# thorstone25/qups

Measured on AMD Instinct MI355X. Metric: beamformed Mpixels/sec (1024^2 px, 256x256 Tx/Rx), higher is better.
Workload: dtype f32; 1 GPU; C3: 256-el FSA (256 Tx x 256 Rx), 1024x1024 ScanCartesian lambda/4, T=2816, complex64, lanczos3; pixels=1048576, pairs_per_frame=68719476736, kernel=tiled, reciprocal_mode=True, reciprocity_fold=True, mirror_mode=True, kernel_name=das_tile_kernel<interp=3,f32,sym,fold,mirror,mb=32,W=128> [jit 56fb2bda29f94d0f], jit=True, fallback_tiles=0, aperture_split=1, parallelism=1 GPU, device=AMD Radeon Graphics (gfx950:sramecc+:xnack-), cu=256

## Files before the change

qups_amd/csrc/das_tile_impl.h:

```cpp
#pragma once
#include "tile_params.h"
#ifndef QDAS_DBG_SYNC
#define QDAS_DBG_SYNC 0
#endif
#ifndef QDAS_ONEACC_PLAIN
#define QDAS_ONEACC_PLAIN 0
#endif
#ifndef QDAS_F16_PIPE
#define QDAS_F16_PIPE 0
#endif
#include "tile_util.h"
#include "tile_taps.h"
#include "tile_hooks.h"
#include "das_tile_cfg.h"

namespace qdas {

typedef __attribute__((address_space(3))) void lds_void;

template <int INTERP_, typename ST_, bool FMOD_, bool WTAB_, bool SYM_, bool FB2_, bool FB4_, int WAVES_, int MB_, int W_, int NBUF_, bool BIG_, bool LUT_, bool BF_ = false, bool MIRQ_ = false, bool FOLD_ = false>
struct TileCfg {
    static constexpr int INTERP = INTERP_, WAVES = WAVES_, MB = MB_, W = W_, NBUF = NBUF_;
    using ST = ST_;
    static constexpr bool FMOD = FMOD_, WTAB = WTAB_, SYM = SYM_, FB2 = FB2_, FB4 = FB4_, BIG = BIG_, LUT = LUT_;
// ... 64 lines not shown
    uint32_t split, S, tile_id;
    uint32_t Sm, sm;
    double fs, symC; int symCi;
    bool tile_interior;
    int need_b;
    static constexpr uint32_t NOT_MINE = 0xffffffffu;
    uint32_t pofs;
    __device__ __forceinline__ bool in_shard() const { return pofs != NOT_MINE; }
    static __device__ __forceinline__ uint32_t lane_now() {
        uint32_t l;
        asm volatile("v_mbcnt_lo_u32_b32 %0, -1, 0\n\tv_mbcnt_hi_u32_b32 %0, -1, %0" : "=v"(l));
        return l;
    }
    uint64_t ipx;
    uint64_t ipx2;
    GT px, py, pz;
    double cf;
    uint32_t n_lo, n_hi, nstage;
    uint32_t nact; bool use_act;
    v2f acc, acc1, acc2, acc3;
    v2f ra[C::MB / 2];
    v2f bw[C::BPIX ? C::MB / 2 : 1]; bool bp;
    double rad[C::F64 ? C::MB : 1];
    double dacc[4];
    v2f tot[C::NFR];
    double dtot[2], w64[2];
    bool wpix, syn;
    int wb[C::WPW], wb2[C::WPW];
    int qo[C::MIRQ ? (C::FOLD ? 2 * C::WPW : 4) : 1];
    uint32_t soff, soff2;
    __amdgpu_buffer_rsrc_t rsD, rsM;
    uint64_t offD, offM, xbytes;
    int fa, fb;

    __device__ __forceinline__ Tile(const TileParams &p) : P(p) {}

    __device__ __forceinline__ void setup(unsigned char *smem);
    __device__ __forceinline__ uint32_t locate(uint32_t &i1, uint32_t &col, bool first, bool image = false);
    template <bool PROBE> __device__ __forceinline__ bool prologue();
    __device__ __forceinline__ void plan_stages();
    template <bool CHECK> __device__ __forceinline__ void run();
    __device__ __forceinline__ void epilogue();

    __device__ __forceinline__ uint32_t blk(uint32_t r) const {
        if constexpr (C::SYM) return (r * S + ((r & 1u) ? S - 1u - split : split)) * C::MB;
        else if constexpr (C::ACT) return (r * Sm + sm) * C::MB;
        else return r * C::MB;
    }
    __device__ __forceinline__ uint32_t nlim(uint32_t m0) const { return C::SYM ? (m0 + C::MB < N ? m0 + C::MB : N) : n_hi; }

    static __device__ __forceinline__ double dsqrt(double d2) {
        const float s0 = __builtin_amdgcn_sqrtf((float)d2);
        const double sd = (double)s0;
        const double r = __builtin_fma(-sd, sd, d2);
        return __builtin_fma(r, (double)(0.5f * __builtin_amdgcn_rcpf(fmaxf(s0, 1.0e-30f))), sd);
    }
    __device__ __forceinline__ double a_of(uint32_t m, const GT *gPv, const GT *gNv) const;
    __device__ __forceinline__ double b_at(GT ex, GT ey, GT ez) const;
    __device__ __forceinline__ double s_at(uint32_t n, GT ex, GT ey, GT ez) const;
    __device__ __forceinline__ bool on_side(uint32_t n, GT ex, GT ey, GT ez) const;
    __device__ __forceinline__ const GT *geo_Pi() const { return (const GT *)P.Pi; }
    __device__ __forceinline__ const GT *geo_Pr() const { return (const GT *)P.Pr; }
    __device__ __forceinline__ const GT *geo_Pv() const { return (const GT *)P.Pv; }
    __device__ __forceinline__ const GT *geo_Nv() const { return (const GT *)P.Nv; }
    struct wraw { uint32_t a, b; };
    __device__ __forceinline__ wraw wload_raw(uint32_t n, bool image = false) const;
    __device__ __forceinline__ v2f wconv(wraw r) const;
    __device__ __forceinline__ v2f wload(uint32_t n) const { return wconv(wload_raw(n)); }

    __device__ __forceinline__ __amdgpu_buffer_rsrc_t make_rs(uint64_t o, uint64_t extra) const;
    __device__ __forceinline__ int wjr(int r) const;
    __device__ __forceinline__ void dma_block(uint32_t m0);
    __device__ __forceinline__ void stage_dma(int bn, int buf);
// ... 265 lines not shown
                }
                act[N] = make_uint2(cnt, 0u);
            }
            __syncthreads();
            nact = (uint32_t)__builtin_amdgcn_readfirstlane((int)act[N].x);
            __syncthreads();
        }
    }
    nstage = 0;
    if (use_act) { for (uint32_t r = 0; blk(r) < M; ++r) nstage += nact; }
    else { for (uint32_t r = 0; blk(r) < M; ++r) nstage += nlim(blk(r)) - n_lo; }
}

template <class C> template <bool CHECK> __device__ __forceinline__ void Tile<C>::run() {
    constexpr int NBUF = C::NBUF, NDMA = C::NDMA;
    auto nsel = [&](uint32_t k) -> uint32_t { if constexpr (C::ACT) { if (use_act) return (uint32_t)__builtin_amdgcn_readfirstlane((int)act[k < N ? k : N - 1].x); } return n_lo + k; };
    auto klim = [&](uint32_t mm) -> uint32_t { if constexpr (C::ACT) { if (use_act) return nact; } return nlim(mm) - n_lo; };
    v2f wcur = {1.f, 0.f}, wcur2 = {1.f, 0.f};
    wraw wnext_r = {0x3f800000u, 0u}, wnext_r2 = {0x3f800000u, 0u};
    const uint32_t n_first = nstage ? nsel(0) : n_lo;
    bool wmir = false;
    if constexpr (C::WMIR) wmir = wpix && QSPEC(MIR, P.mir) && QSPEC(HAS_APIX, P.apix != nullptr) && QSPEC(GEN_KIND, P.gen_kind) == 0;
    auto wload64 = [&](uint32_t nn, double &wr, double &wi) {
        const uint64_t k = ipx + (P.apix_pixel_only ? 0ull : P.I1 * P.I2 * P.I3 * (uint64_t)nn);
        if (P.apix_real) { wr = ((const double *)P.apix)[k]; wi = 0.0; }
        else { const double2 v = ((const double2 *)P.apix)[k]; wr = v.x; wi = v.y; }
    };
    double w64n[2] = {1.0, 0.0};
    if constexpr (C::W64) { if (wpix) wload64(n_first, w64[0], w64[1]); }
    else if (wpix) { wcur = wload(n_first); wcur2 = wcur; if constexpr (C::WMIR) { if (wmir) wcur2 = wconv(wload_raw(n_first, true)); } }
    float tbc = 0.f, tbn = 0.f;
    const uint64_t Ilut = P.i_begin + P.i_count;
    if constexpr (C::LUT) tbc = P.lut_rx[ipx + Ilut * n_first];
    uint32_t pr = 0, pk = 0, pm0 = blk(0);
    dma_block(pm0);
    auto rec_base = [&](uint32_t k) -> float { if constexpr (C::F64) return __int_as_float(nrec64[k].b); else return nrec[k].x; };
    float vbn; uint32_t vpn;
    auto front_entry = [&](uint32_t kk) {
        if constexpr (C::ACT) {
            if (use_act) { const uint2 e = act[kk < N ? kk : N - 1]; vpn = e.x; vbn = __uint_as_float(e.y); return; }
        }
        const uint32_t q = n_lo + kk;
        vpn = q; vbn = rec_base(q < N ? q : N - 1);
    };
    front_entry(0);
    int dbn = 0; uint32_t dpn = 0;
    auto dma_prep = [&]() {
        dbn = __builtin_amdgcn_readfirstlane(__float_as_int(vbn));
        dpn = (uint32_t)__builtin_amdgcn_readfirstlane((int)vpn);
        front_entry(pk + 1 == klim(pm0) ? 0u : pk + 1);
    };
    auto dma_go = [&](int buf) {
        if constexpr (C::ACT) {
            if (use_act) {
                soff = ((dpn >> P.stage_shift) - (n_lo >> P.stage_shift)) * (uint32_t)strN * (uint32_t)C::SB;
                if constexpr (C::WMIR) { if (QSPEC(MIR, P.mir)) soff2 = (n_hi - 1u - dpn) * (uint32_t)strN * (uint32_t)C::SB; }
            }
        }
        stage_dma(dbn, buf);
        if (++pk == klim(pm0)) { pk = 0; pm0 = blk(++pr); dma_block(pm0); }
    };
    auto dma_next = [&](int buf) { dma_prep(); dma_go(buf); };
    constexpr uint32_t WBUF = 2u * C::MB * 8u + 16u;
    float2 wnx = {0.f, 0.f};
    auto wst_load = [&](uint32_t nn, uint32_t mm0) {
        if constexpr (C::WST) {
// ... 19 lines not shown
#pragma unroll
    for (int b = 0; b < NBUF - 1; ++b)
        if ((uint32_t)b < nstage) dma_next(b);
    if (nstage >= (uint32_t)(NBUF - 1)) asm volatile("s_waitcnt vmcnt(%0)\n\ts_barrier" ::"n"((NBUF - 2) * NDMA) : "memory");
    else asm volatile("s_waitcnt vmcnt(0)\n\ts_barrier" ::: "memory");
    int buf = 0;
    uint32_t cr = 0, k = 0, n = n_first, m0 = blk(0);
    for (uint32_t st = 0; st < nstage; ++st) {
        timer.mark(0);
        if constexpr ((QDAS_DBG_SYNC & 1) != 0) __syncthreads();
        const bool more = st + (NBUF - 1) < nstage;
        const uint32_t n_next = (NBUF == 2 && C::ACT) ? (uint32_t)__builtin_amdgcn_readfirstlane((int)vpn) : nsel(k + 1 == klim(m0) ? 0u : k + 1);
        const bool skip = wpix && (__ballot(wcur.x != 0.f || wcur.y != 0.f || (C::WMIR && (wcur2.x != 0.f || wcur2.y != 0.f))) == 0ull);
        int rec_b; GT rec_x, rec_y, rec_z;
        if constexpr (C::F64) { const rec64 r = nrec64[n]; rec_b = r.b; rec_x = r.x; rec_y = r.y; rec_z = r.z; }
        else { const float4 r = nrec[n]; rec_b = __float_as_int(r.x); rec_x = r.y; rec_y = r.z; rec_z = r.w; }
        float phB = 0.f;
        if constexpr (C::FMOD && !C::F64) {
            phB = Bext[n];
            if constexpr (C::MIRQ) phB = __uint_as_float((uint32_t)__builtin_amdgcn_readfirstlane((int)__float_as_uint(phB)));
        }
        uint64_t wmask = ~0ull, xmask = ~0ull;
        if constexpr (C::WST) {
            const uint4 mk = *(const uint4 *)(wst + (uint32_t)buf * WBUF + 2 * C::MB * 8);
            wmask = (uint64_t)(uint32_t)__builtin_amdgcn_readfirstlane((int)mk.x) | ((uint64_t)(uint32_t)__builtin_amdgcn_readfirstlane((int)mk.y) << 32);
            if constexpr (C::SYM) xmask = (uint64_t)(uint32_t)__builtin_amdgcn_readfirstlane((int)mk.z) | ((uint64_t)(uint32_t)__builtin_amdgcn_readfirstlane((int)mk.w) << 32);
        }
        const bool dma_late = C::SYM && !hooks::no_late_dma && wave < C::WAVES / 2;
        const bool dma_now = !hooks::no_stage_dma && more && !dma_late;
        if (dma_now) dma_prep();
        if constexpr (C::W64) { if (wpix && st + 1 < nstage) wload64(n_next, w64n[0], w64n[1]); }
        else if (wpix && st + 1 < nstage) { wnext_r = wload_raw(n_next); if constexpr (C::WMIR) { if (wmir) wnext_r2 = wload_raw(n_next, true); } }
        if constexpr (C::LUT) { if (st + 1 < nstage) tbn = P.lut_rx[ipx + Ilut * n_next]; }
        if (st + 1 < nstage) wst_load(n_next, k + 1 == klim(m0) ? blk(cr + 1) : m0);
        if (dma_now) dma_go((buf + NBUF - 1) % NBUF);
        if constexpr ((QDAS_DBG_SYNC & 32) != 0) asm volatile("s_waitcnt vmcnt(0) lgkmcnt(0)" ::: "memory");
        if constexpr ((QDAS_DBG_SYNC & 2) != 0) { asm volatile("s_waitcnt vmcnt(0) lgkmcnt(0)" ::: "memory"); __syncthreads(); }
        timer.mark(1);
        if constexpr (C::F64) {
            if (k == 0) {
#pragma unroll
                for (int p = 0; p < C::MB; ++p) {
                    const uint32_t ma = m0 + p < M ? m0 + p : M - 1;
                    rad[p] = block_residual64(px, py, pz, cf, fs, kindB, (lds_cdouble *)PvL, (lds_cdouble *)NvL, ma, Abase[ma], tapinfo<C::INTERP>::OFF);
                    __builtin_amdgcn_sched_barrier(0);
                }
            }
        } else if (k == 0) {
#pragma unroll
            for (int p = 0; p < C::MB / 2; ++p) {
                const uint32_t ma = m0 + 2 * p < M ? m0 + 2 * p : M - 1, mb = m0 + 2 * p + 1 < M ? m0 + 2 * p + 1 : M - 1;
                if constexpr (C::SYM) {
                    const float4 ea = nrec[ma], eb = nrec[mb];
                    const double fc = symC - (double)symCi - 0.5;
                    ra[p] = (v2f){(float)(b_at(ea.y, ea.z, ea.w) - (double)__float_as_int(ea.x) + fc),
                                  (float)(b_at(eb.y, eb.z, eb.w) - (double)__float_as_int(eb.x) + fc)};
                } else if constexpr (C::LUT)
                    ra[p] = (v2f){(float)(a_of(ma, nullptr, nullptr) - ((double)Abase[ma] + 0.5)), (float)(a_of(mb, nullptr, nullptr) - ((double)Abase[mb] + 0.5))};
                else
                    ra[p] = (v2f){block_residual(px, py, pz, cf, fs, kindB, (lds_cfloat *)PvL, (lds_cfloat *)NvL, ma, Abase[ma], tapinfo<C::INTERP>::OFF),
                                  block_residual(px, py, pz, cf, fs, kindB, (lds_cfloat *)PvL, (lds_cfloat *)NvL, mb, Abase[mb], tapinfo<C::INTERP>::OFF)};
                __builtin_amdgcn_sched_barrier(0);
            }
            if constexpr (C::BPIX) {
                if (!bp) {
#pragma unroll
                    for (int p = 0; p < C::MB / 2; ++p) bw[p] = (v2f){1.f, 1.f};
                } else {
                    const uint64_t Itot = P.I1 * P.I2 * P.I3;
                    uint32_t ip32 = (uint32_t)ipx;
                    asm volatile("" : "+v"(ip32));
#pragma unroll
                    for (int p = 0; p < C::MB / 2; ++p) {
                        const uint32_t ma = m0 + 2 * p < M ? m0 + 2 * p : M - 1, mb = m0 + 2 * p + 1 < M ? m0 + 2 * p + 1 : M - 1;
                        const float *rowa = P.bpix + Itot * ma, *rowb = P.bpix + Itot * mb;
                        asm volatile("" : "+s"(rowa), "+s"(rowb));
                        bw[p] = (v2f){rowa[ip32], rowb[ip32]};
                        __builtin_amdgcn_sched_barrier(0);
                    }
                }
            }
        }
        timer.mark(2);
        if constexpr ((QDAS_DBG_SYNC & 4) != 0) __syncthreads();
        if constexpr (C::F64) {
            const int bn = rec_b;
            const double rbd = s_at(n, rec_x, rec_y, rec_z) - (double)bn;
            const uint32_t cbase = win_off + (uint32_t)buf * (C::NW * C::WB);
            bool skip64 = false;
            if constexpr (C::W64) skip64 = wpix && __ballot(w64[0] != 0.0 || w64[1] != 0.0) == 0ull;
            if (skip64) {}
            else if (m0 + C::MB <= M) pairs_f64<CHECK, false>(n, m0, bn, rbd, cbase);
            else                      pairs_f64<CHECK, true>(n, m0, bn, rbd, cbase);
        } else if (!skip) {
            const int bn = rec_b;
            const float rb = C::LUT ? tbc - (float)bn : hooks::fake_rx_delay ? (float)(lane * 2 + 3) + 0.37f * (float)(n & 7)
                                                                            : (float)(s_at(n, rec_x, rec_y, rec_z) - (double)bn);
            const uint32_t cbase = win_off + (uint32_t)buf * (C::NW * C::WB) - (MAGIC_BITS * (uint32_t)C::SB);
            if (C::SYM ? (n < m0 && (!C::FOLD || m0 + C::MB <= M)) : (m0 + C::MB <= M)) {
                if constexpr (C::TWO && (C::F32 || C::SYM || QDAS_F16_PIPE) && C::K == 4 && !(CHECK || C::FMOD || C::WTAB) && !hooks::no_pipeline && !((QDAS_ONEACC_PLAIN || C::INTERP == 3) && C::ONEACC))
                    pairs_pipelined(rb, cbase);
                else
                {
                    constexpr uint64_t FULL = C::MB >= 64 ? ~0ull : ((1ull << (C::MB & 63)) - 1ull);
                    bool done = false;
                    if constexpr (C::WST) {
                        if (wmask == FULL && (!C::SYM || xmask == FULL)) {
                            pairs_plain<CHECK, false, false>(n, m0, bn, rb, cbase, phB, wst_off + (uint32_t)buf * WBUF, wmask, xmask);
                            done = true;
                        }
                    }
                    if (!done) pairs_plain<CHECK, false>(n, m0, bn, rb, cbase, phB, wst_off + (uint32_t)buf * WBUF, wmask, xmask);
                }
            } else {
                pairs_plain<CHECK, true>(n, m0, bn, rb, cbase, phB, wst_off + (uint32_t)buf * WBUF, wmask, xmask);
            }
        }
        if constexpr ((QDAS_DBG_SYNC & 8) != 0) __syncthreads();
        if constexpr (!hooks::no_fair_prio) __builtin_amdgcn_s_setprio(3);
        if (!hooks::no_stage_dma && more && dma_late) dma_next((buf + NBUF - 1) % NBUF);
        if (st + 1 < nstage) wst_store((buf + 1) % NBUF);
        timer.mark(3);
        if (!hooks::no_stage_barrier) {
            if (more) asm volatile("s_waitcnt vmcnt(%0) lgkmcnt(0)\n\ts_barrier" ::"n"((NBUF - 2) * NDMA) : "memory");
            else asm volatile("s_waitcnt vmcnt(0) lgkmcnt(0)\n\ts_barrier" ::: "memory");
        }
        timer.mark(4);
        timer.stage_done();
        buf = (buf + 1 == NBUF) ? 0 : buf + 1;
        if (syn) {
// ... 5 lines not shown
                if (in_shard()) {
                    float2 *plane = (float2 *)P.y + (size_t)f * P.y_fstride + (size_t)n * P.y_ld;
                    asm volatile("" : "+s"(plane));
                    uint32_t po = pofs;
                    asm volatile("" : "+v"(po));
                    float *q = (float *)(plane + po);
                    unsafeAtomicAdd(q, Sf[f].x); unsafeAtomicAdd(q + 1, Sf[f].y);
                }
            }
            if (wpix) { if constexpr (!C::F32) asm volatile("" : "+v"(wnext_r.a)); wcur = wconv(wnext_r); }
            acc = acc1 = acc2 = acc3 = (v2f){0.f, 0.f};
        } else if (C::W64 && wpix) {
            if constexpr (C::W64) {
                const double sr = dacc[0] + dacc[2], si = dacc[1] + dacc[3];
                dtot[0] += w64[0] * sr - w64[1] * si; dtot[1] += w64[0] * si + w64[1] * sr;
                dacc[0] = dacc[1] = dacc[2] = dacc[3] = 0.0;
                w64[0] = w64n[0]; w64[1] = w64n[1];
            }
        } else if (wpix) {
            v2f Sf[4];
            frame_sums(Sf);
#pragma unroll
            for (int f = 0; f < C::NFR; ++f) {
                const v2f wf = (C::WMIR && f == 1) ? wcur2 : wcur;
                tot[f] += (v2f){wf.x * Sf[f].x - wf.y * Sf[f].y, wf.x * Sf[f].y + wf.y * Sf[f].x};
            }
            acc = acc1 = acc2 = acc3 = (v2f){0.f, 0.f};
            if constexpr (!C::F32) asm volatile("" : "+v"(wnext_r.a));
            wcur = wconv(wnext_r);
            wcur2 = wcur;
            if constexpr (C::WMIR) { if (wmir) { asm volatile("" : "+v"(wnext_r2.a)); wcur2 = wconv(wnext_r2); } }
        }
        if constexpr (C::LUT) tbc = tbn;
        if (++k == klim(m0)) { k = 0; m0 = blk(++cr); }
        n = n_next;
    }
}

template <class C> __device__ __forceinline__ void Tile<C>::epilogue() {
    if (syn || C::BF) return;
    if constexpr (C::F64) {
        if (pofs != NOT_MINE) {
            uint32_t po = pofs;
            asm volatile("" : "+v"(po));
            ST *base = S > 1 ? (ST *)P.part + (size_t)split * P.i_count : (ST *)P.y;
            asm volatile("" : "+s"(base));
            if (C::W64 && wpix) st(base, (size_t)po, cplx<double>{dtot[0], dtot[1]});
            else st(base, (size_t)po, cplx<double>{dacc[0] + dacc[2], dacc[1] + dacc[3]});
        }
    } else {
        v2f res[4];
        frame_sums(res);
        uint32_t po = pofs;
        if constexpr (C::SYM) { uint32_t i1, col; po = locate(i1, col, false); }
        if constexpr (C::FOLDQ && C::FB2) {
            uint32_t i1, col;
            const uint32_t po2 = locate(i1, col, false, true);
            const uint32_t pos[2] = {po, po2};
#pragma unroll
            for (int f = 0; f < 2; ++f) {
#pragma unroll
                for (int h = 0; h < 2; ++h) {
                    uint32_t q = pos[h];
                    if (q == NOT_MINE) continue;
                    asm volatile("" : "+v"(q));
                    const v2f r = res[2 * f + h];
// ... 12 lines not shown
                for (int f = 0; f < 2; ++f) {
                    uint32_t q = pos[f];
                    if (q == NOT_MINE) continue;
                    asm volatile("" : "+v"(q));
                    v2f r = res[f];
                    if constexpr (!C::MIRQ) { if (wpix) r = tot[f]; }
                    if (S > 1) { float2 *base = P.part + (size_t)split * (P.i_count << (QSPEC(MIR, P.mir) == 2 ? 1 : 0)); asm volatile("" : "+s"(base)); base[q] = make_float2(r.x, r.y); }
                    else { ST *base = (ST *)P.y; asm volatile("" : "+s"(base)); st(base, (size_t)q, cplx<float>{r.x, r.y}); }
                }
                return;
            }
        }
        if (po != NOT_MINE) {
            asm volatile("" : "+v"(po));
#pragma unroll
            for (int f = 0; f < C::NFR; ++f) {
                const v2f r = wpix ? tot[f] : res[f];
                if (S > 1) { float2 *base = P.part + ((size_t)split * C::NFR + f) * P.i_count; asm volatile("" : "+s"(base)); base[po] = make_float2(r.x, r.y); }
                else { ST *base = (ST *)P.y + (size_t)f * P.y_fstride; asm volatile("" : "+s"(base)); st(base, (size_t)po, cplx<float>{r.x, r.y}); }
            }
        }
    }
}

template <class C, bool PROBE> __device__ __forceinline__ void das_tile_body(const TileParams &P, unsigned char *smem) {
    Tile<C> t(P);
    t.timer.begin();
    t.setup(smem);
    if (!t.template prologue<PROBE>()) return;
    if constexpr (!PROBE) {
        t.timer.prologue_done();
        t.plan_stages();
        if (P.pro_mask == 2) return;
        if (t.tile_interior) t.template run<false>(); else t.template run<true>();
        t.timer.finish(t.lane, t.wave, C::WAVES);
        t.epilogue();
    }
}

template <int INTERP, typename ST, bool FMOD, bool WTAB, bool SYM, bool FB2, bool FB4, int WAVES, int MB, int W, int NBUF, int PSZ, int BPC, bool PROBE, bool BIG = false, bool LUT = false, bool BFM = false, bool MIRQ = false, bool FOLD = false>
__global__ void __launch_bounds__(WAVES * 64, WAVES * BPC / 4)
das_tile_kernel(const TileParams P) {
    static_assert(PSZ == 16, "16-byte DMA pieces");
    extern __shared__ __attribute__((aligned(16))) unsigned char smem[];
    das_tile_body<TileCfg<INTERP, ST, FMOD, WTAB, SYM, FB2, FB4, WAVES, MB, W, NBUF, BIG, LUT, BFM, MIRQ, FOLD>, PROBE>(P, smem);
}

#ifndef __HIPCC_RTC__
}
#include "jit.h"
namespace qdas {
void tile_census(int ci, int interp, int sample_bytes, bool fm, bool wt, bool probe);
bool tile_prepare_only();
template <int INTERP, typename ST, int CI>
static hipError_t launch_tile_i(const TileParams &P, unsigned ntiles, size_t lds, hipStream_t s) {
    constexpr Cfg G = CFGS[CI];
    constexpr bool FOLD = (CI >= 17 && CI <= 21);
    constexpr bool MIRQ = (CI == 15 || CI == 16 || CI == 17 || CI == 18 || CI == 20);
    constexpr bool SYM = (CI == 1 || CI == 7 || CI == 8 || MIRQ || FOLD), FB2 = (CI == 3 || CI == 4 || CI == 20 || CI == 21), FB4 = (CI == 5 || CI == 6), BIG = (CI == 9), LUT = (CI == 10 || CI == 11), BFM = (CI == 12);
    const bool fm = P.fmod != 0.0, wt = P.wtab != nullptr;
    const dim3 g(ntiles * (P.probe ? 1u : P.ksplit)), b(G.waves * 64);
    tile_census(CI, INTERP, (int)sizeof(ST), fm, wt, P.probe != 0);
#define QDAS_LAUNCH(FM, WT) QDAS_LAUNCH_P(FM, WT, false)
#define QDAS_LAUNCH_P(FM, WT, PR)                                                                        \
    do {                                                                                                 \
        if constexpr (tile_prebuilt(CI, INTERP, FM, WT, PR)) {                                           \
// ... 56 lines not shown
```

qups_amd/csrc/qdas_api.hip:

```cpp
#include <hip/hip_runtime.h>
#include <hip/hip_fp16.h>

#include <algorithm>
#include <cmath>
#include <cstdarg>
#include <cstdio>
#include <cstdlib>
#include <cstring>
#include <string>
#include <mutex>
#include <vector>

#include "../../include/qdas.h"
#include "qdas_kernels.h"
#include "jit.h"

using namespace qdas;

static thread_local std::string g_err;

static int fail(int code, const char *fmt, ...) {
    char buf[512];
    va_list ap;
    va_start(ap, fmt);
// ... 28 lines not shown
    int prev = -1;
    bool restore = false;
    hipError_t err = hipSuccess;
    explicit DeviceGuard(int dev) {
        if (dev < 0) return;
        err = hipGetDevice(&prev);
        if (err == hipSuccess && prev != dev) { err = hipSetDevice(dev); restore = err == hipSuccess; }
    }
    ~DeviceGuard() { if (restore) (void)hipSetDevice(prev); }
    DeviceGuard(const DeviceGuard &) = delete;
    DeviceGuard &operator=(const DeviceGuard &) = delete;
};

static size_t real_size(int dtype) { return dtype == QDAS_F64 ? 8 : 4; }
static size_t data_size(int dtype) { return dtype == QDAS_F64 ? 16 : (dtype == QDAS_F32 ? 8 : 4); }
static size_t apod_real_size(int dtype) { return dtype == QDAS_F64 ? 8 : (dtype == QDAS_F32 ? 4 : 2); }

struct qdas_plan {
    qdas_desc d{};
    uint64_t I = 0, i_count = 0, y_ld = 0, oN = 1, oM = 1;
    double cinv0 = 0.0;
    int device = 0;
    int kernel = QDAS_KERNEL_GENERIC;
    std::vector<void *> owned;
    GenericParams gp{};
    TileParams tp{};
    TileConfig tc{};
    unsigned ntiles = 0, tile_cols = 0;
    bool no_fallback = false;
    double misfit_frac = 0.0;
    bool wtab_real = false;
    void *fold_buf = nullptr;
    const void *fold_wtab = nullptr;
    double mirror_bound = -1.0, recip_bound = -1.0;
    bool prefolded = false;
    qdas_plan *f16_child = nullptr;
    void *y32 = nullptr;
    bool fb2_ok = false;
    bool fb4_off = false;
    bool fold2_ok = false;
    void *fold_buf2 = nullptr;
    qdas_plan *frames_twin = nullptr;
    bool twin_tried = false;
    uint32_t *fallback = nullptr;
    size_t jit_lds = 0;
    int jit_mb = 0, jit_w = 0;
    int hint_mb = 0, hint_w = 0;
    hipFunction_t jit_fn = nullptr;
    std::string jit_tag;
    bool prep2 = false, prep4 = false;
    bool timing = false;
    hipEvent_t e0 = nullptr, e1 = nullptr;
    float last_ms = 0.f;
    void *dx = nullptr, *dy = nullptr;
    size_t x_bytes = 0, y_bytes = 0;
    void *dx2 = nullptr, *dy2 = nullptr;
    hipStream_t copy_stream = nullptr;
    hipEvent_t ex[2] = {nullptr, nullptr}, ek[2] = {nullptr, nullptr};

    ~qdas_plan() {
        if (frames_twin) qdas_plan_destroy(frames_twin);
        if (f16_child) qdas_plan_destroy(f16_child);
        for (void *p : owned) (void)hipFree(p);
        if (e0) (void)hipEventDestroy(e0);
        if (e1) (void)hipEventDestroy(e1);
        for (int k = 0; k < 2; ++k) { if (ex[k]) (void)hipEventDestroy(ex[k]); if (ek[k]) (void)hipEventDestroy(ek[k]); }
// ... 929 lines not shown
    t.pro_mask = 0;
    const bool with_mask = t.act_bytes != 0 && !getenv("QDAS_NO_PRO_MASK");
    const size_t stride = 2 * ((size_t)t.M + t.N) + 8 + (with_mask ? (t.N + 31) / 32 : 0), bytes = (size_t)pl->ntiles * stride * sizeof(float);
    if (bytes > (1ull << 30)) return QDAS_OK;
    void *buf = nullptr;
    if (hipMalloc(&buf, bytes) != hipSuccess) { (void)hipGetLastError(); return QDAS_OK; }
    pl->owned.push_back(buf);
    TileParams p = t;
    p.probe = 1; p.x = nullptr; p.y = nullptr; p.wtab = nullptr; p.apix = nullptr; p.pro_out = (float *)buf; p.pro_mask = with_mask ? 1 : 0;
    HIPCHK(hipMemsetAsync(buf, 0, bytes, 0));
    const hipError_t e = launch_tile(p, pl->d.sz.dtype, pl->ntiles, nullptr);
    if (e != hipSuccess) { (void)hipGetLastError(); return QDAS_OK; }
    HIPCHK(hipStreamSynchronize(nullptr));
    HIPCHK(hipMemset(pl->fallback, 0, sizeof(uint32_t)));
    t.pro_tab = (const float *)buf;
    t.pro_mask = with_mask ? 3 : 0;
    return QDAS_OK;
}

static void plan_cache_activity(qdas_plan *pl) {
    TileParams &t = pl->tp;
    if (pl->kernel != QDAS_KERNEL_TILED || t.pro_mask != 3) return;
    TileParams p = t;
    p.nfr = 1; p.x = nullptr; p.y = nullptr; p.ksplit = 1; p.ksplit_m = 1; p.part = nullptr; p.pro_mask = 2; p.pro_out = const_cast<float *>(t.pro_tab);
    const std::string keep = g_err;
    hipError_t e = launch_tile(p, pl->d.sz.dtype, pl->ntiles, nullptr, pl->jit_fn, pl->jit_lds);
    if (e == hipSuccess) e = hipStreamSynchronize(nullptr);
    if (e == hipSuccess && !pl->no_fallback) e = hipMemset(pl->fallback, 0, sizeof(uint32_t));
    g_err = keep;
    if (e == hipSuccess) t.pro_mask = 1;
    else { (void)hipGetLastError(); t.pro_mask = 0; t.pro_tab = nullptr; }
}

static int plan_build_tiled(qdas_plan *pl, const qdas_desc *desc, PlanBuild &b) {
    int rc;
    if ((rc = plan_setup_tile_params(pl, desc, b))) return rc;
    if ((rc = plan_pixel_weights(pl, desc, b))) return rc;
    if ((rc = plan_weight_table(pl, desc, b))) return rc;
    if ((rc = plan_probe_chain(pl, desc, b))) return rc;
    if ((rc = plan_side_split(pl, desc, b))) return rc;
    if ((rc = plan_wide_windows(pl, desc, b))) return rc;
    if ((rc = plan_stage_shape(pl, desc, b))) return rc;
    if ((rc = plan_split_aperture(pl, b))) return rc;
    if ((rc = plan_cache_prologue(pl))) return rc;
    b.outcome.ksplit = pl->tp.ksplit;
    const modes::LaunchShape model = modes::derive_launch_shape(*desc, b.rq, b.sy, b.outcome), built = launch_shape(pl->tp, pl->d.sz.dtype, false);
    if (const char *f = modes::shape_mismatch(model, built))
        return fail(QDAS_EINVAL, "internal: the built plan differs from the mode model of plan_modes.h in '%s' -- please report the descriptor", f);
    return QDAS_OK;
}

static int plan_create_impl(qdas_plan *pl, qdas_plan **out, const qdas_desc *desc, bool *replaced) {
    *replaced = false;
    int rc = plan_init(pl, desc);
    if (rc) return rc;
    const qdas_sizes &z = pl->d.sz;
    DeviceGuard guard(desc->device);
    if (guard.err != hipSuccess) return fail(QDAS_EHIP, "hipSetDevice(%d): %s", desc->device, hipGetErrorString(guard.err));
    { hipError_t e = hipGetDevice(&pl->device); if (e != hipSuccess) return fail(QDAS_EHIP, "hipGetDevice: %s", hipGetErrorString(e)); }
    if (pl->I == 0 || z.N == 0 || z.M == 0) return QDAS_OK;
    if ((desc->plan_flags & QDAS_PLAN_PREFOLDED) && z.S > 0)
        return fail(QDAS_EUNSUPPORTED, "QDAS_PLAN_PREFOLDED: apodization arrays belong to the fold (qdas_fold_desc.wtab), not to the plan that is handed folded frames");
    PlanBuild b;
    b.desc = desc;
    b.sw = read_switches();
    if ((rc = plan_import_inputs(pl, desc, b))) return rc;
    if ((rc = plan_resolve_modes(pl, desc, b))) return rc;
    if (pl->kernel == QDAS_KERNEL_TILED && (rc = plan_build_tiled(pl, desc, b))) return rc;
    const bool mslab = (desc->plan_flags & QDAS_PLAN_MIRROR_SLAB) != 0;
    if (mslab && !(pl->kernel == QDAS_KERNEL_TILED && pl->tp.mir == 2))
        return fail(QDAS_EUNSUPPORTED, "QDAS_PLAN_MIRROR_SLAB: the lateral-mirror mode is not available for this problem (geometry not mirror-symmetric "
                                       "about x = 0, weights / modes it does not take, or tiles that do not fit the staging windows): use plain slabs");
    int remake = 0;
    if ((rc = plan_jit(pl, desc, &remake))) return rc;
    if (remake) {
        qdas_desc d2 = *desc;
        d2.plan_flags |= remake;
        const std::string keep = g_err;
        *replaced = true;
        const int rc2 = qdas_plan_create(out, &d2);
        if (rc2 == QDAS_OK) g_err = keep;
        return rc2;
    }
    if (pl->prefolded && pl->kernel == QDAS_KERNEL_TILED && !pl->no_fallback)
        return fail(QDAS_EUNSUPPORTED, "QDAS_PLAN_PREFOLDED: tiles of this image do not fit the staging windows (they would be redone from the unfolded frame)");
    plan_f16_child(pl, desc);
    bool no_compiler = false;
    plan_resolve_kernel(pl, &no_compiler);
    if (no_compiler) {
        const std::string why = g_err;
        if (desc->kernel == QDAS_KERNEL_TILED || mslab || pl->prefolded) return fail(QDAS_EUNSUPPORTED, "%s", why.c_str());
        qdas_desc d2 = *desc;
        d2.kernel = QDAS_KERNEL_GENERIC;
        *replaced = true;
        const int rc2 = qdas_plan_create(out, &d2);
        if (rc2 == QDAS_OK) g_err = why + " -- using the generic kernel";
        return rc2;
    }
    plan_cache_activity(pl);
    return plan_finish(pl, desc, b);
}

extern "C" int qdas_plan_create(qdas_plan **out, const qdas_desc *desc) {
    if (!out || !desc) return fail(QDAS_EINVAL, "null argument");
    *out = nullptr;
    int rc = validate(desc);
    if (rc) return rc;
    qdas_plan *pl = new qdas_plan();
    bool replaced = false;
    rc = plan_create_impl(pl, out, desc, &replaced);
    if (rc || replaced) { delete pl; return rc; }
    *out = pl;
    return QDAS_OK;
}

extern "C" void qdas_plan_destroy(qdas_plan *pl) {
    if (!pl) return;
    DeviceGuard guard(pl->device);
    delete pl;
}

extern "C" int qdas_plan_kernel(const qdas_plan *pl) { return pl ? pl->kernel : 0; }

extern "C" int qdas_plan_fallback_tiles(const qdas_plan *pl, uint64_t *n) {
    if (!pl || !n) return fail(QDAS_EINVAL, "null argument");
    if (pl->f16_child) return qdas_plan_fallback_tiles(pl->f16_child, n);
    *n = 0;
    if (pl->kernel != QDAS_KERNEL_TILED || !pl->fallback) return QDAS_OK;
    uint32_t c = 0;
    HIPCHK(hipMemcpy(&c, pl->fallback, sizeof c, hipMemcpyDeviceToHost));
    *n = c;
    return QDAS_OK;
}

extern "C" int qdas_plan_tile_shape(const qdas_plan *pl, int *tile_z, int *tile_cols, int *wave_z, int *ksplit) {
    if (!pl || !tile_z || !tile_cols) return fail(QDAS_EINVAL, "null argument");
    if (pl->f16_child) return qdas_plan_tile_shape(pl->f16_child, tile_z, tile_cols, wave_z, ksplit);
    const bool tiled = pl->kernel == QDAS_KERNEL_TILED;
    *tile_z = tiled ? (1 << pl->tp.tz_log2) : 0;
    *tile_cols = tiled ? (int)pl->tile_cols : 0;
    if (wave_z) *wave_z = tiled ? (1 << pl->tp.wz_log2) : 0;
    if (ksplit) *ksplit = tiled ? (int)pl->tp.ksplit : 0;
    return QDAS_OK;
}

extern "C" int qdas_plan_mirror(const qdas_plan *pl) { if (pl && pl->f16_child) return qdas_plan_mirror(pl->f16_child); return pl && pl->kernel == QDAS_KERNEL_TILED && pl->tp.mir ? 1 : 0; }

extern "C" int qdas_plan_reciprocal(const qdas_plan *pl) { return pl && pl->kernel == QDAS_KERNEL_TILED && pl->tp.sym ? 1 : 0; }

extern "C" int qdas_plan_symmetry_bound(const qdas_plan *pl, double *mirror_samples, double *reciprocal_samples) {
    if (!pl) return fail(QDAS_EINVAL, "null plan");
    if (pl->f16_child) return qdas_plan_symmetry_bound(pl->f16_child, mirror_samples, reciprocal_samples);
    const bool tiled = pl->kernel == QDAS_KERNEL_TILED;
    if (mirror_samples) *mirror_samples = (tiled && pl->tp.mir) ? pl->mirror_bound : -1.0;
    if (reciprocal_samples) *reciprocal_samples = (tiled && pl->tp.sym) ? pl->recip_bound : -1.0;
    return QDAS_OK;
}

extern "C" int qdas_plan_folded(const qdas_plan *pl) { if (pl && pl->f16_child) return 1; return pl && pl->kernel == QDAS_KERNEL_TILED && pl->tp.fold ? 1 : 0; }

extern "C" int qdas_fold(const qdas_fold_desc *d, const void *x, void *xs, void *stream) {
    if (!d || !x || !xs) return fail(QDAS_EINVAL, "null argument");
    if (d->dtype != QDAS_F32 && d->dtype != QDAS_F16) return fail(QDAS_EINVAL, "qdas_fold: complex64 or complex32 (fp16) frames");
    if (d->N > 65535) return fail(QDAS_EUNSUPPORTED, "qdas_fold: at most 65535 elements");
    DeviceGuard guard(d->device);
    HIPCHK(guard.err);
    HIPCHK(launch_fold(x, xs, d->wtab, d->T, d->N, d->strN ? d->strN : d->T, d->strM ? d->strM : d->T * d->N, (hipStream_t)stream, d->dtype == QDAS_F16));
    return QDAS_OK;
}

extern "C" int qdas_plan_kernel_name(const qdas_plan *pl, char *buf, size_t len) {
    if (!pl || !buf || !len) return fail(QDAS_EINVAL, "null argument");
    if (pl->f16_child) {
        char tmp[256];
        int rc = qdas_plan_kernel_name(pl->f16_child, tmp, sizeof tmp);
        if (rc) return rc;
        std::string nm(tmp);
        const size_t at = nm.find(",f32");
        if (at != std::string::npos) nm.replace(at, 4, ",f16>f32");
        if (pl->fold_wtab && nm.find(",wtab") == std::string::npos) { const size_t f = nm.find(",fold"); if (f != std::string::npos) nm.insert(f + 5, ",wtab"); }
        snprintf(buf, len, "%s", nm.c_str());
        return QDAS_OK;
    }
    const qdas_sizes &z = pl->d.sz;
    const char *dts = z.dtype == QDAS_F64 ? "f64" : (z.dtype == QDAS_F32 ? "f32" : "f16");
    if (pl->kernel == QDAS_KERNEL_TILED) {
        const TileParams &t = pl->tp;
        snprintf(buf, len, "das_tile_kernel<interp=%d,%s%s%s%s%s%s%s,mb=%d,W=%d> [%s]", z.flag & 7, dts, t.sym ? ",sym" : "", t.fold ? ",fold" : "", t.fmod != 0.0 ? ",fmod" : "",
                 (t.wtab || (t.fold && pl->fold_wtab)) ? ",wtab" : "", t.big ? ",big" : "", t.mir ? ",mirror" : ((t.St && !t.syn) ? ",roles swapped" : ""), pl->jit_fn ? pl->jit_mb : pl->tc.mb, (pl->jit_fn && pl->jit_w) ? pl->jit_w : pl->tc.window, pl->jit_tag.empty() ? "prebuilt" : pl->jit_tag.c_str());
    } else snprintf(buf, len, "das_generic_kernel<interp=%d,%s>", z.flag & 7, dts);
    return QDAS_OK;
}

extern "C" int qdas_plan_set_timing(qdas_plan *pl, int enable) {
    if (!pl) return fail(QDAS_EINVAL, "null plan");
    pl->timing = enable != 0;
    if (pl->timing && !pl->e0) { HIPCHK(hipEventCreate(&pl->e0)); HIPCHK(hipEventCreate(&pl->e1)); }
    return QDAS_OK;
}

extern "C" int qdas_plan_last_kernel_ms(const qdas_plan *pl, float *ms) {
    if (!pl || !ms) return fail(QDAS_EINVAL, "null argument");
    *ms = pl->last_ms;
    return QDAS_OK;
}

static int hip_rc(hipError_t e) { HIPCHK(e); return QDAS_OK; }

static int run_frame(qdas_plan *pl, const void *x, void *y, hipStream_t s, int nf = 1, uint64_t x_fstride = 0, uint64_t y_fstride = 0) {
    const qdas_sizes &z = pl->d.sz;
    if (pl->f16_child && nf == 1) {
        const TileParams &c = pl->f16_child->tp;
        HIPCHK(launch_fold(x, pl->fold_buf, pl->fold_wtab, z.T, z.N, c.strN, c.strM, s, 1));
        int rc = run_frame(pl->f16_child, pl->fold_buf, pl->y32, s);
        if (rc) return rc;
        HIPCHK(launch_y32_to_y16(pl->y32, y, pl->f16_child->y_ld, s));
        return QDAS_OK;
    }
    if (pl->kernel == QDAS_KERNEL_TILED) {
        TileParams t = pl->tp;
        t.x = x; t.y = y;
        t.nfr = nf; t.x_fstride = x_fstride; t.y_fstride = y_fstride;
        if (t.fold && pl->prefolded) {
            if (!pl->no_fallback) return fail(QDAS_EUNSUPPORTED, "QDAS_PLAN_PREFOLDED: tiles of this image do not fit the staging windows and would need the unfolded frame");
        } else if (t.fold) {
            HIPCHK(launch_fold(x, pl->fold_buf, pl->fold_wtab, z.T, z.N, t.strN, t.strM, s));
            t.x = pl->fold_buf;
            if (nf == 2) {
                if (!pl->fold_buf2) return fail(QDAS_EINVAL, "internal: no second fold buffer");
                HIPCHK(launch_fold((const char *)x + x_fstride, pl->fold_buf2, pl->fold_wtab, z.T, z.N, t.strN, t.strM, s));
                t.x_fstride = (uint64_t)((intptr_t)pl->fold_buf2 - (intptr_t)pl->fold_buf);
            }
        }
        if (t.syn) {
            const size_t ds = data_size(z.dtype);
            for (int f = 0; f < nf; ++f)
                HIPCHK(hipMemset2DAsync((char *)y + (size_t)f * y_fstride * ds, (size_t)pl->y_ld * ds, 0, (size_t)pl->i_count * ds, pl->oN * pl->oM, s));
        }
        const hipFunction_t jf = nf == 1 ? pl->jit_fn : nullptr;
        if (pl->no_fallback) return hip_rc(launch_tile(t, z.dtype, pl->ntiles, s, jf, pl->jit_lds));
        HIPCHK(hipMemsetAsync(pl->fallback, 0, sizeof(uint32_t), s));
        HIPCHK(launch_tile(t, z.dtype, pl->ntiles, s, jf, pl->jit_lds));
        GenericParams g = pl->gp;
        g.x = x; g.y = y; g.y_ld = pl->y_ld;
        g.tile_list = pl->fallback;
        g.tile_cols = pl->tile_cols;
        g.tile_zl = (uint32_t)pl->tp.tz_log2;
        g.blocks_per_tile = (64 * pl->tc.waves + 255) / 256;
        g.tiles_z = pl->tp.tiles_z;
        HIPCHK(launch_generic(g, z.dtype, pl->ntiles * g.blocks_per_tile, s));
        for (int f = 1; f < nf; ++f) {
            g.x = (const char *)x + (size_t)f * x_fstride; g.y = (char *)y + (size_t)f * y_fstride * data_size(z.dtype);
            HIPCHK(launch_generic(g, z.dtype, pl->ntiles * g.blocks_per_tile, s));
        }
    } else {
// ... 807 lines not shown
```

qups_amd/csrc/tile_params.h:

```cpp
#pragma once
#include "tile_rtc.h"

namespace qdas {

struct TileParams {
    const float *Pi, *Pr, *Pv, *Nv, *St;
    int32_t kindB, kindS;
    int32_t stage_shift;
    const void *x;
    void *y;
    const void *wtab;
    const void *apix;
    int32_t apix_real;
    int32_t apix_pixel_only;
    int32_t gen_kind;
    double gen_p0, gen_p1;
    const float *rxn;
    uint32_t act_bytes;
    uint64_t T, N, M, I1, I2, I3;
    uint64_t i_begin, i_count;
    uint64_t strN, strM;
    double cinv_fs;
    const float *cinv_pix;
    double fs, fmod;
    int32_t flag, VS, DV;
    int32_t narrow;
    int32_t big;
    int32_t sym;
    int32_t tz_log2;
    int32_t wz_log2;
    int32_t probe;
    uint32_t tiles_z, tiles_x, tile_x0;
    int32_t syn;
    uint64_t y_ld;
    int32_t bf;
    uint64_t bf_pn, bf_pm;
    int32_t nfr;
    uint64_t x_fstride, y_fstride;
    uint32_t ksplit;
    float2 *part;
    uint32_t *fallback_list;
    uint32_t fallback_cap;
    const float *lut_tx, *lut_rx;
    const float *bpix;
    int32_t mir;
    int32_t fold;
    const float *pro_tab;
    float *pro_out;
    int32_t pro_mask;
    uint32_t ksplit_m;
    int32_t probe_w;
};

}
```

qups_amd/csrc/tile_prologue.h:

```cpp
#pragma once

namespace qdas {

template <class C> template <bool PROBE> __device__ __forceinline__ bool Tile<C>::prologue() {
    constexpr int WAVES = C::WAVES, THREADS = C::THREADS, K = C::K, INTERP = C::INTERP;
    constexpr bool SYM = C::SYM, LUT = C::LUT;
    using GT = typename C::GT;
    const GT *gPv = geo_Pv(), *gNv = geo_Nv(), *gPr = geo_Pr();
    constexpr uint32_t PCH = QDAS_PROLOGUE_CHUNK;
    const uint32_t MX = (M > N ? M : N) < PCH ? (M > N ? M : N) : PCH;
    const uint64_t Ilut = P.i_begin + P.i_count;
    const bool has_st = QSPEC(HAS_ST, P.St != nullptr);
    float a_lo = INFINITY, a_hi = -INFINITY, a_ext = 0.f;
    const size_t pro_stride = 2 * ((size_t)M + N) + 8 + (P.pro_mask ? (N + 31) / 32 : 0);
    const uint32_t tile_slot = tile_id - P.tiles_z * P.tile_x0;
    const float *ptab = nullptr;
    if constexpr (!PROBE && !LUT) { if (P.pro_tab) ptab = P.pro_tab + (size_t)tile_slot * pro_stride; }
    float b_lo = INFINITY, b_hi = -INFINITY, b_ext = 0.f;
    if (ptab) {
        if constexpr (!SYM) {
            for (uint32_t m = tid; m < M; m += THREADS) { Abase[m] = __float_as_int(ptab[2 * m]); Aext[m] = ptab[2 * m + 1]; }
        }
        for (uint32_t n = tid; n < N; n += THREADS) {
            const float bb = ptab[2 * ((size_t)M + n)], e = ptab[2 * ((size_t)M + n) + 1];
// ... 121 lines not shown
                o[2 * ((size_t)M + n)] = bb; o[2 * ((size_t)M + n) + 1] = Bext[n];
            }
            if (tid == 0) { float *q = o + 2 * ((size_t)M + N); q[0] = a_lo; q[1] = b_lo; q[2] = a_hi; q[3] = b_hi; q[4] = a_ext; q[5] = b_ext; }
        }
    }
    if (!(a_ext + b_ext + (float)(K + 1) <= (float)((PROBE && P.probe_w > 0) ? P.probe_w : C::W))) {
        if (tid == 0 && split == 0) {
            const uint32_t slot = atomicAdd(&P.fallback_list[0], 1u);
            if (slot < P.fallback_cap) P.fallback_list[1 + slot] = tile_id;
        }
        return false;
    }
    if constexpr (PROBE) return false;
    tile_interior = (a_lo + b_lo >= 1.0f) && (a_hi + b_hi + (float)(K + 1) < (float)T);
#ifdef QDAS_DMA_TRIM
    need_b = __builtin_amdgcn_readfirstlane((((int)(a_ext + b_ext) + K + 3) * (int)C::SB + 15) & ~15);
    if (need_b > (int)C::WB) need_b = (int)C::WB;
#else
    need_b = (int)C::WB;
#endif
    if constexpr (C::FMOD && !C::F64) {
        const double f = P.fmod / fs;
        for (uint32_t m = tid; m < M; m += THREADS) { const double c = ((double)Abase[m] + 0.5 - tapinfo<INTERP>::OFF) * f; Aext[m] = (float)(c - floor(c)); }
        for (uint32_t n = tid; n < N; n += THREADS) { const double c = (double)__float_as_int(nrec[n].x) * f; Bext[n] = (float)(c - floor(c)); }
    }
    if constexpr (!LUT) {
        for (uint32_t k = tid; k < 4 * M; k += THREADS) PvL[k] = gPv[k];
        for (uint32_t k = tid; k < 3 * M; k += THREADS) NvL[k] = gNv[k];
    }
    __syncthreads();
    return true;
}

}
```

Before: 72.14 Mpixel/s.

## Precompute per-tile receive residual delays into a global table for folded kernels

```diff
diff --git a/qups_amd/csrc/das_tile_impl.h b/qups_amd/csrc/das_tile_impl.h
--- a/qups_amd/csrc/das_tile_impl.h
+++ b/qups_amd/csrc/das_tile_impl.h
@@ -120,6 +120,8 @@
     __amdgpu_buffer_rsrc_t rsD, rsM;
     uint64_t offD, offM, xbytes;
     int fa, fb;
+    static constexpr uint32_t RBLD = 1024;
+    const float *rbp;
 
     __device__ __forceinline__ Tile(const TileParams &p) : P(p) {}
 
@@ -127,6 +129,7 @@
     __device__ __forceinline__ uint32_t locate(uint32_t &i1, uint32_t &col, bool first, bool image = false);
     template <bool PROBE> __device__ __forceinline__ bool prologue();
     __device__ __forceinline__ void plan_stages();
+    __device__ __forceinline__ void fill_rb();
     template <bool CHECK> __device__ __forceinline__ void run();
     __device__ __forceinline__ void epilogue();
 
@@ -458,6 +461,9 @@
     float tbc = 0.f, tbn = 0.f;
     const uint64_t Ilut = P.i_begin + P.i_count;
     if constexpr (C::LUT) tbc = P.lut_rx[ipx + Ilut * n_first];
+    float rbc = 0.f, rbn = 0.f;
+    auto rb_load = [&](uint32_t nn) -> float { return rbp[(size_t)nn * RBLD + ((uint32_t)wave * 64u + lane_now())]; };
+    if constexpr (C::FOLD) { if (rbp && nstage) rbc = rb_load(n_first); }
     uint32_t pr = 0, pk = 0, pm0 = blk(0);
     dma_block(pm0);
     auto rec_base = [&](uint32_t k) -> float { if constexpr (C::F64) return __int_as_float(nrec64[k].b); else return nrec[k].x; };
@@ -543,6 +549,7 @@
         if constexpr (C::W64) { if (wpix && st + 1 < nstage) wload64(n_next, w64n[0], w64n[1]); }
         else if (wpix && st + 1 < nstage) { wnext_r = wload_raw(n_next); if constexpr (C::WMIR) { if (wmir) wnext_r2 = wload_raw(n_next, true); } }
         if constexpr (C::LUT) { if (st + 1 < nstage) tbn = P.lut_rx[ipx + Ilut * n_next]; }
+        if constexpr (C::FOLD) { if (rbp && st + 1 < nstage) rbn = rb_load(n_next); }
         if (st + 1 < nstage) wst_load(n_next, k + 1 == klim(m0) ? blk(cr + 1) : m0);
         if (dma_now) dma_go((buf + NBUF - 1) % NBUF);
         if constexpr ((QDAS_DBG_SYNC & 32) != 0) asm volatile("s_waitcnt vmcnt(0) lgkmcnt(0)" ::: "memory");
@@ -605,8 +612,10 @@
             else                      pairs_f64<CHECK, true>(n, m0, bn, rbd, cbase);
         } else if (!skip) {
             const int bn = rec_b;
-            const float rb = C::LUT ? tbc - (float)bn : hooks::fake_rx_delay ? (float)(lane * 2 + 3) + 0.37f * (float)(n & 7)
-                                                                            : (float)(s_at(n, rec_x, rec_y, rec_z) - (double)bn);
+            float rb;
+            if (C::FOLD && rbp) rb = rbc;
+            else rb = C::LUT ? tbc - (float)bn : hooks::fake_rx_delay ? (float)(lane * 2 + 3) + 0.37f * (float)(n & 7)
+                                                                      : (float)(s_at(n, rec_x, rec_y, rec_z) - (double)bn);
             const uint32_t cbase = win_off + (uint32_t)buf * (C::NW * C::WB) - (MAGIC_BITS * (uint32_t)C::SB);
             if (C::SYM ? (n < m0 && (!C::FOLD || m0 + C::MB <= M)) : (m0 + C::MB <= M)) {
                 if constexpr (C::TWO && (C::F32 || C::SYM || QDAS_F16_PIPE) && C::K == 4 && !(CHECK || C::FMOD || C::WTAB) && !hooks::no_pipeline && !((QDAS_ONEACC_PLAIN || C::INTERP == 3) && C::ONEACC))
@@ -678,6 +687,7 @@
             if constexpr (C::WMIR) { if (wmir) { asm volatile("" : "+v"(wnext_r2.a)); wcur2 = wconv(wnext_r2); } }
         }
         if constexpr (C::LUT) tbc = tbn;
+        if constexpr (C::FOLD) rbc = rbn;
         if (++k == klim(m0)) { k = 0; m0 = blk(++cr); }
         n = n_next;
     }
@@ -756,6 +766,7 @@
         t.timer.prologue_done();
         t.plan_stages();
         if (P.pro_mask == 2) return;
+        t.fill_rb();
         if (t.tile_interior) t.template run<false>(); else t.template run<true>();
         t.timer.finish(t.lane, t.wave, C::WAVES);
         t.epilogue();
diff --git a/qups_amd/csrc/qdas_api.hip b/qups_amd/csrc/qdas_api.hip
--- a/qups_amd/csrc/qdas_api.hip
+++ b/qups_amd/csrc/qdas_api.hip
@@ -84,6 +84,8 @@
     bool wtab_real = false;
     void *fold_buf = nullptr;
     const void *fold_wtab = nullptr;
+    size_t rb_bytes = 0;
+    float *rb_tab = nullptr;
     double mirror_bound = -1.0, recip_bound = -1.0;
     bool prefolded = false;
     qdas_plan *f16_child = nullptr;
@@ -1079,6 +1081,19 @@
     else { (void)hipGetLastError(); t.pro_mask = 0; t.pro_tab = nullptr; }
 }
 
+static void plan_residual_table(qdas_plan *pl) {
+    const TileParams &t = pl->tp;
+    if (pl->kernel != QDAS_KERNEL_TILED || !t.fold || t.ksplit != 1 || !pl->ntiles || getenv("QDAS_NO_RB_TAB")) return;
+    const uint64_t mb = (pl->jit_fn && pl->jit_mb) ? (uint64_t)pl->jit_mb : (uint64_t)pl->tc.mb;
+    if (mb == 0 || (t.M < 4 * mb && !getenv("QDAS_RB_TAB"))) return;
+    const size_t bytes = (size_t)pl->ntiles * t.N * 1024 * sizeof(float);
+    if (bytes > (1ull << 30)) return;
+    void *buf = nullptr;
+    if (hipMalloc(&buf, bytes) != hipSuccess) { (void)hipGetLastError(); return; }
+    pl->owned.push_back(buf);
+    pl->rb_tab = (float *)buf; pl->rb_bytes = bytes;
+}
+
 static int plan_build_tiled(qdas_plan *pl, const qdas_desc *desc, PlanBuild &b) {
     int rc;
     if ((rc = plan_setup_tile_params(pl, desc, b))) return rc;
@@ -1145,6 +1160,7 @@
         return rc2;
     }
     plan_cache_activity(pl);
+    plan_residual_table(pl);
     return plan_finish(pl, desc, b);
 }
 
@@ -1204,6 +1220,7 @@
     return QDAS_OK;
 }
 
+extern "C" unsigned long long qdas_debug_plan_residual_table(const qdas_plan *pl) { if (pl && pl->f16_child) pl = pl->f16_child; return pl && pl->rb_tab ? (unsigned long long)pl->rb_bytes : 0ull; }
 extern "C" int qdas_plan_folded(const qdas_plan *pl) { if (pl && pl->f16_child) return 1; return pl && pl->kernel == QDAS_KERNEL_TILED && pl->tp.fold ? 1 : 0; }
 
 extern "C" int qdas_fold(const qdas_fold_desc *d, const void *x, void *xs, void *stream) {
@@ -1268,6 +1285,7 @@
         TileParams t = pl->tp;
         t.x = x; t.y = y;
         t.nfr = nf; t.x_fstride = x_fstride; t.y_fstride = y_fstride;
+        if (pl->rb_tab && t.fold && nf == 1 && t.ksplit == 1) t.rbtab = pl->rb_tab;
         if (t.fold && pl->prefolded) {
             if (!pl->no_fallback) return fail(QDAS_EUNSUPPORTED, "QDAS_PLAN_PREFOLDED: tiles of this image do not fit the staging windows and would need the unfolded frame");
         } else if (t.fold) {
diff --git a/qups_amd/csrc/tile_params.h b/qups_amd/csrc/tile_params.h
--- a/qups_amd/csrc/tile_params.h
+++ b/qups_amd/csrc/tile_params.h
@@ -50,6 +50,7 @@
     int32_t pro_mask;
     uint32_t ksplit_m;
     int32_t probe_w;
+    float *rbtab;
 };
 
 }
diff --git a/qups_amd/csrc/tile_prologue.h b/qups_amd/csrc/tile_prologue.h
--- a/qups_amd/csrc/tile_prologue.h
+++ b/qups_amd/csrc/tile_prologue.h
@@ -177,4 +177,19 @@
     return true;
 }
 
+template <class C> __device__ __forceinline__ void Tile<C>::fill_rb() {
+    rbp = nullptr;
+    if constexpr (C::FOLD && !hooks::fake_rx_delay) {
+        if (!P.rbtab) return;
+        float *o = P.rbtab + (size_t)blockIdx.x * N * RBLD;
+        asm volatile("" : "+s"(o));
+        rbp = o;
+        const uint32_t slot = (uint32_t)wave * 64u + (uint32_t)lane;
+        for (uint32_t n = 0; n < N; ++n) {
+            const float4 r = nrec[n];
+            o[(size_t)n * RBLD + slot] = (float)(s_at(n, r.y, r.z, r.w) - (double)__float_as_int(r.x));
+        }
+    }
 }
+
+}
```

Measured after the change: 70.88 Mpixel/s. -1.8%, worse.
